# Rutgers-ECE-MML4SS/multimodal-sensor-fusion-with-attention-RajeevAtla

Measured on AMD Instinct MI355X. Metric: HybridFusion fwd+bwd samples/sec at 1/2/4/8 MI355X; CPU-ref parity, higher is better.
Workload: dtype fp32; 1 GPU; c2: HybridFusion M=3 B=256/gpu L=128 D=128 H=128 heads=4 C=5 dropout=0.1 train, fwd+CE(ls=0.05)+bwd+clip(1.0)+AdamW; fused step (flat buffers, one hipGraph); global_batch=256, per_gpu_batch=256, seq_len=128, parallelism=dp1, graph=True, matmul_precision=highest

## Files before the change

multimodal-sensor-fusion-with-attention-rajeevatla_amd/csrc/gemm.hip:

```cpp
#include <algorithm>
#include <cstdlib>
#include <cstring>
#include <map>
#include <vector>

#include "mmf_device.h"

namespace mmf {

namespace {

constexpr int BM = 128, BN = 128, BK = 32, NT = 256;
#ifndef MMF_GEMM_DK
#define MMF_GEMM_DK 16
#endif
#ifndef MMF_GEMM_NS
#define MMF_GEMM_NS 3
#endif
constexpr int LDS_STRIDE = BM + 4;
constexpr int LDS_STRIDE_T = BM + 1;

typedef float f32x4 __attribute__((ext_vector_type(4)));

struct TileCtx {
// ... 1206 lines not shown
  const GemmGroup& g = J.g;
  if (amode != MODE_KR || bmode != MODE_KR || J.nsrc != 1 || !(g.epi & EPI_PARTIAL)) return false;
  if (g.seg_rows > 0 || J.src[0].a.seg_stride || J.src[0].b.seg_stride) return false;
  const int64_t n = (int64_t)(g.nbatch < 1 ? 1 : g.nbatch) * g.nsplit * g.M * (g.N + 1);
  return n <= (1 << 20) && g.kchunk <= 256;
}

struct ReduceArgs {
  ReduceJob j[48];
  int32_t njobs;
};

__global__ __launch_bounds__(256) void partial_reduce_kernel(const ReduceArgs a) {
  ReduceJob J = a.j[blockIdx.y];
  const int64_t MN = (int64_t)J.M * J.N;
  const int batch = blockIdx.z;
  if (batch >= J.nbatch) return;
  J.part += (int64_t)batch * J.nsplit * MN;
  if (J.part_db) J.part_db += (int64_t)batch * J.nsplit * J.M;
  J.out += (int64_t)batch * J.bs_out;
  if (J.db) J.db += (int64_t)batch * J.bs_db;
  __shared__ f32x4 red[4][64];
  const int el = threadIdx.x & 63, sg = threadIdx.x >> 6;
  const bool v4 = (MN % 4) == 0 && ((uintptr_t)J.part & 15) == 0;
  const int64_t n4 = v4 ? MN / 4 : MN;
  const bool out_al = ((uintptr_t)J.out & 15) == 0;
  for (int64_t c0 = (int64_t)blockIdx.x * 64; c0 < n4; c0 += (int64_t)gridDim.x * 64) {
    const int64_t col = c0 + el;
    f32x4 s0 = {0.f, 0.f, 0.f, 0.f}, s1 = s0, s2 = s0, s3 = s0;
    if (col < n4) {
      if (v4) {
        const f32x4* base = reinterpret_cast<const f32x4*>(J.part) + col;
        const int64_t st = MN / 4;
        int k = sg;
#pragma unroll 4
        for (; k + 12 < J.nsplit; k += 16) {
          s0 += base[(int64_t)k * st];
          s1 += base[(int64_t)(k + 4) * st];
          s2 += base[(int64_t)(k + 8) * st];
          s3 += base[(int64_t)(k + 12) * st];
        }
        for (; k < J.nsplit; k += 4) s0 += base[(int64_t)k * st];
      } else {
        for (int k = sg; k < J.nsplit; k += 4) s0[0] += J.part[(int64_t)k * MN + col];
      }
    }
    __syncthreads();
    red[sg][el] = (s0 + s1) + (s2 + s3);
    __syncthreads();
    if (sg == 0 && col < n4) {
      const f32x4 r = (red[0][el] + red[1][el]) + (red[2][el] + red[3][el]);
      if (!v4) J.out[col] = r[0];
      else if (out_al) reinterpret_cast<f32x4*>(J.out)[col] = r;
      else {
        float* o = J.out + col * 4;
        o[0] = r[0]; o[1] = r[1]; o[2] = r[2]; o[3] = r[3];
      }
    }
  }
  if (J.db && (J.part_db || J.nsplit == 0) && blockIdx.x == gridDim.x - 1) {
    __shared__ float redb[4][64];
    for (int i0 = 0; i0 < J.M; i0 += 64) {
      const int i = i0 + el;
      float s0 = 0.f, s1 = 0.f, s2 = 0.f, s3 = 0.f;
      if (i < J.M) {
        int k = sg;
#pragma unroll 4
        for (; k + 12 < J.nsplit; k += 16) {
          s0 += J.part_db[(int64_t)k * J.M + i];
          s1 += J.part_db[(int64_t)(k + 4) * J.M + i];
          s2 += J.part_db[(int64_t)(k + 8) * J.M + i];
          s3 += J.part_db[(int64_t)(k + 12) * J.M + i];
        }
        for (; k < J.nsplit; k += 4) s0 += J.part_db[(int64_t)k * J.M + i];
      }
      __syncthreads();
      redb[sg][el] = (s0 + s1) + (s2 + s3);
      __syncthreads();
      if (sg == 0 && i < J.M) J.db[i] = (redb[0][el] + redb[1][el]) + (redb[2][el] + redb[3][el]);
    }
  }
}

__global__ __launch_bounds__(256) void mask_dropout_rows_kernel(const MaskDropArgs a) {
  const int m = blockIdx.x;
  const bool drop = a.p > 0.f && (a.rng != nullptr || a.rng_live != nullptr);
  RngSnap rs{0, 0};
  {
    const uint64_t* src = a.rng_live ? a.rng_live : (drop ? reinterpret_cast<const uint64_t*>(a.rng) : nullptr);
    if (src) {
      rs.seed = src[0];
      rs.offset = src[1];
    }
  }
  const uint32_t thr = p16(a.p);
  if (m >= a.n) {
    const MaskDropArgs::KeepWordJob& K = a.kw[m - a.n];
    const uint32_t nkt = K.Lk >> 5;
    const uint32_t nwords = (uint32_t)a.B * (uint32_t)a.heads * K.Lq * nkt;
    for (uint32_t i = blockIdx.y * 256u + threadIdx.x; i < nwords; i += gridDim.y * 256u) {
      const uint32_t row = (nkt & (nkt - 1)) == 0 ? i >> (31 - __builtin_clz(nkt)) : i / nkt;
      const uint32_t kt = i - row * nkt;
      const uint64_t blk0 = ((uint64_t)row * K.Lk + 32 * kt) >> 3;
      uint32_t bits = 0;
#pragma unroll
      for (int g = 0; g < 4; ++g) {
        const uint4 rr = philox_block(rs, K.site, blk0 + g);
        const uint32_t wv[4] = {rr.x, rr.y, rr.z, rr.w};
#pragma unroll
        for (int k = 0; k < 4; ++k) {
          bits |= ((wv[k] & 0xFFFFu) >= thr ? 1u : 0u) << (8 * g + 2 * k);
          bits |= ((wv[k] >> 16) >= thr ? 1u : 0u) << (8 * g + 2 * k + 1);
        }
      }
      K.bits[(uint64_t)row * K.kw_ld + kt] = bits;
    }
    return;
  }
  const MaskDropJob& J = a.j[m];
  const int64_t n = J.rows * J.D;
  const float inv_keep = a.p < 1.f ? 1.f / (1.f - a.p) : 0.f;
  const int D = J.D, L = J.L, M = a.M;
  for (int64_t blk = (int64_t)blockIdx.y * blockDim.x + threadIdx.x; blk * 8 < n;
       blk += (int64_t)gridDim.y * blockDim.x) {
    uint4 r = make_uint4(0, 0, 0, 0);
    if (drop) r = philox_block(rs, J.site, (uint64_t)blk);
    const int64_t base = blk * 8;
    if (J.vec && base + 8 <= n) {
      const float sc = a.mask[(base / D / L) * M + m];
      const float4 v0 = *reinterpret_cast<const float4*>(J.x + base);
      const float4 v1 = *reinterpret_cast<const float4*>(J.x + base + 4);
      float o[8] = {v0.x, v0.y, v0.z, v0.w, v1.x, v1.y, v1.z, v1.w};
#pragma unroll
      for (int e = 0; e < 8; ++e) {
        float v = o[e] * sc;
        if (drop) v = keep_from(r, e, thr) ? v * inv_keep : 0.f;
        o[e] = v;
      }
      if (J.outb) {
        bf16x8 pk;
#pragma unroll
        for (int e = 0; e < 8; ++e) pk[e] = (__bf16)o[e];
        *reinterpret_cast<bf16x8*>(reinterpret_cast<__bf16*>(J.out) + base) = pk;
      } else {
        *reinterpret_cast<float4*>(J.out + base) = make_float4(o[0], o[1], o[2], o[3]);
        *reinterpret_cast<float4*>(J.out + base + 4) = make_float4(o[4], o[5], o[6], o[7]);
      }
    } else {
      for (int e = 0; e < 8 && base + e < n; ++e) {
        const int64_t idx = base + e;
        float v = J.x[idx] * a.mask[(idx / D / L) * M + m];
        if (drop) v = keep_from(r, e, thr) ? v * inv_keep : 0.f;
        if (J.outb) reinterpret_cast<__bf16*>(J.out)[idx] = (__bf16)v;
        else J.out[idx] = v;
      }
    }
  }
  if (a.rng_snap && blockIdx.x == 0 && blockIdx.y == 0 && threadIdx.x == 0) *a.rng_snap = rs;
}

bool dma_ok(const Operand& op, int mode, int eext, int bstride, int nbatch) {
  if (!op.vec || op.row_div < 1) return false;
  if (nbatch > 1 && (bstride % 4) != 0) return false;
  if (mode == MODE_KR && (eext % 4) != 0) return false;
  return true;
}

bool job_fast(const GemmJob& J, int amode, int bmode) {
  const GemmGroup& g = J.g;
  const int nb = g.nbatch < 1 ? 1 : g.nbatch;
  if ((g.epi & EPI_PARTIAL) && (g.kchunk % 32) != 0) return false;
  for (int s = 0; s < J.nsrc; ++s) {
    const GemmSrc& src = J.src[s];
    if ((src.K % 4) != 0 || !dma_ok(src.a, amode, g.M, g.bs_a, nb) || !dma_ok(src.b, bmode, g.N, g.bs_b, nb))
      return false;
  }
  return true;
}

}

namespace {

inline bool aligned16(const void* p) { return ((uintptr_t)p & 15) == 0; }

bool job_wsr(const GemmJob& J, int amode, int bmode) {
  const GemmGroup& g = J.g;
  if (amode != MODE_RK || (bmode != MODE_RK && bmode != MODE_KR) || J.nsrc != 1 || g.nbatch > 1) return false;
  if (g.epi & ~(EPI_BIAS | EPI_RELU | EPI_DROP | EPI_COLSUM | EPI_ROWSCALE)) return false;
  static const bool ext_on = getenv("MMF_WSR_EPI") != nullptr;
  if (!ext_on && (bmode != MODE_RK || (g.epi & ~(EPI_BIAS | EPI_RELU)))) return false;
  if ((g.epi & EPI_ROWSCALE) && (g.rs_div <= 0 || g.rs_div % BM != 0 || !g.rowscale)) return false;
  if ((g.epi & EPI_COLSUM) && !g.colsum) return false;
  const GemmSrc& s = J.src[0];
  const bool b_ok = bmode == MODE_RK ? (s.b.ld % 4 == 0 && aligned16(s.b.ptr)) : s.b.ld >= g.N;
  return g.N == BN && g.M % BM == 0 && s.K % WSR_DK == 0 && s.K >= WSR_DK && s.K <= 8 * WSR_NKC &&
         s.a.row_div == 1 && s.b.row_div == 1 && s.a.ld % 4 == 0 && aligned16(s.a.ptr) && b_ok &&
         s.a.seg_stride == 0 && s.b.seg_stride == 0 && g.ldc % 4 == 0 && aligned16(g.C);
}

int cu_count() {
  static int n = 0;
  if (n == 0) {
    int dev = 0;
    if (hipGetDevice(&dev) != hipSuccess ||
        hipDeviceGetAttribute(&n, hipDeviceAttributeMultiprocessorCount, dev) != hipSuccess || n <= 0)
      n = 256;
  }
  return n;
}

hipError_t launch_wsr(const GemmJob* jobs, int njobs, hipStream_t st, uint64_t* rng_advance, int bmode, float drop_p,
                      const RngSnap* rng) {
  for (int done = 0; done < njobs;) {
    GemmArgs args;
    memset(&args, 0, sizeof(args));
    args.amode = MODE_RK;
    args.bmode = bmode;
    args.drop_p = drop_p;
    args.rng = rng;
    args.rng_advance = rng_advance;
    rng_advance = nullptr;
    int ng = 0, items = 0;
    double fl = 0.0, by = 0.0;
    while (done < njobs && ng < GEMM_MAX_GROUPS) {
      GemmGroup g = jobs[done].g;
      g.nbatch = 1;
      g.src_begin = ng;
      g.src_count = 1;
      args.s[ng] = jobs[done].src[0];
      args.tile_off[ng] = items;
      args.g[ng++] = g;
      items += g.M / BM;
      fl += 2.0 * g.M * g.N * jobs[done].src[0].K;
      by += 4.0 * ((double)g.M + g.N) * jobs[done].src[0].K + 4.0 * g.M * g.N;
      ++done;
    }
// ... 468 lines not shown
      GemmGroup g = J.g;
      g.nbatch = 1;
      g.src_begin = ns;
      g.src_count = J.nsrc;
      for (int s = 0; s < J.nsrc; ++s) args.s[ns++] = J.src[s];
      const bool partial = (g.epi & EPI_PARTIAL) != 0;
      args.tile_off[ng] = max_blocks;
      args.g[ng++] = g;
      max_blocks += ((g.M + BM - 1) / BM) * ((g.N + bn - 1) / bn) * (partial ? g.nsplit : 1);
      ++done;
    }
    args.ngroups = ng;
    if (ilv_on && ng > 1) {
      const int T = args.tile_off[1];
      bool even = T > 0 && T % 8 == 0;
      for (int gi = 1; gi < ng && even; ++gi)
        even = (gi + 1 < ng ? args.tile_off[gi + 1] : max_blocks) - args.tile_off[gi] == T;
      args.ilv = even ? 1 : 0;
    }
    double fl = 0.0, by = 0.0;
    for (int gi = 0; gi < ng; ++gi) {
      const GemmGroup& g = args.g[gi];
      const bool partial = (g.epi & EPI_PARTIAL) != 0;
      for (int si = g.src_begin; si < g.src_begin + g.src_count; ++si) {
        fl += 2.0 * g.M * g.N * args.s[si].K;
        by += 2.0 * ((double)g.M + g.N) * args.s[si].K;
      }
      by += partial ? 4.0 * g.nsplit * g.M * g.N
                    : ((g.epi & EPI_BF16) ? 2.0 : 4.0) * g.M * g.N + ((g.epi & EPI_BF16COPY) ? 2.0 * g.M * g.N : 0.0);
    }
    static const char* const kName[4] = {"", "gemm_lds_kernel<0, 0, 32, 3, 1, 1>", "gemm_lds_kernel<1, 1, 32, 3, 1, 2>",
                                         "gemm_lds_kernel<0, 1, 32, 3, 1, 3>"};
    static const char* const kNameW[4] = {"", "", "gemm_lds_kernel<1, 1, 32, 3, 1, 2, 1>",
                                          "gemm_lds_kernel<0, 1, 32, 3, 1, 3, 1>"};
    ProfLaunch prof_(st, wide ? kNameW[form] : kName[form], fl, by);
    if (form == 1) mmf_launch((gemm_lds_kernel<MODE_RK, MODE_RK, 32, 3, 1, 1>), dim3(max_blocks, 1), dim3(NT), 0, st, args);
    else if (form == 2 && wide) mmf_launch((gemm_lds_kernel<MODE_KR, MODE_KR, 32, 3, 1, 2, 1>), dim3(max_blocks, 1), dim3(NT), 0, st, args);
    else if (form == 2) mmf_launch((gemm_lds_kernel<MODE_KR, MODE_KR, 32, 3, 1, 2>), dim3(max_blocks, 1), dim3(NT), 0, st, args);
    else if (wide) mmf_launch((gemm_lds_kernel<MODE_RK, MODE_KR, 32, 3, 1, 3, 1>), dim3(max_blocks, 1), dim3(NT), 0, st, args);
    else mmf_launch((gemm_lds_kernel<MODE_RK, MODE_KR, 32, 3, 1, 3>), dim3(max_blocks, 1), dim3(NT), 0, st, args);
    const hipError_t e = hipGetLastError();
    if (e != hipSuccess) return e;
  }
  return hipSuccess;
}

hipError_t launch_reduce(const ReduceJob* jobs, int njobs, hipStream_t st) {
  int done = 0;
  while (done < njobs) {
    ReduceArgs a;
    memset(&a, 0, sizeof(a));
    int n = 0;
    int64_t maxmn = 0;
    int maxbatch = 1;
    while (done < njobs && n < 48) {
      a.j[n] = jobs[done++];
      if (a.j[n].nbatch < 1) a.j[n].nbatch = 1;
      if (a.j[n].nbatch > maxbatch) maxbatch = a.j[n].nbatch;
      const int64_t mn = (int64_t)a.j[n].M * a.j[n].N;
      if (mn > maxmn) maxmn = mn;
      ++n;
    }
    a.njobs = n;
    int blocks = (int)((maxmn / 4 + 63) / 64);
    if (blocks < 1) blocks = 1;
    if (blocks > 4096) blocks = 4096;
    for (int i = 0; i < n; ++i)
      if (a.j[i].db && (a.j[i].part_db || a.j[i].nsplit == 0)) { ++blocks; break; }
    double by = 0.0;
    for (int i = 0; i < n; ++i) {
      const ReduceJob& r = a.j[i];
      by += 4.0 * r.nbatch * ((double)r.nsplit + 1) * r.M * ((double)r.N + (r.part_db ? 1 : 0));
    }
    ProfLaunch prof_(st, "partial_reduce_kernel", 0.0, by);
    mmf_launch(partial_reduce_kernel, dim3(blocks, n, maxbatch), dim3(256), 0, st, a);
    hipError_t e = hipGetLastError();
    if (e != hipSuccess) return e;
  }
  return hipSuccess;
}

hipError_t launch_mask_dropout(MaskDropArgs a, hipStream_t st) {
  if (a.n < 1 || a.n > 8 || a.nkw < 0 || a.nkw > 16) return hipErrorInvalidValue;
  int64_t maxblk = 1;
  for (int m = 0; m < a.n; ++m) {
    MaskDropJob& J = a.j[m];
    J.vec = (J.D % 8) == 0 && ((uintptr_t)J.x & 15) == 0 && ((uintptr_t)J.out & 15) == 0;
    maxblk = std::max<int64_t>(maxblk, (J.rows * J.D + 7) / 8);
  }
  double by = 0.0;
  for (int m = 0; m < a.n; ++m) by += (a.j[m].outb ? 6.0 : 8.0) * a.j[m].rows * a.j[m].D;
  for (int i = 0; i < a.nkw; ++i) {
    const int64_t nw = (int64_t)a.B * a.heads * a.kw[i].Lq * (a.kw[i].Lk / 32);
    if (a.kw[i].Lk % 32 != 0 || nw >= ((int64_t)1 << 31)) return hipErrorInvalidValue;
    maxblk = std::max<int64_t>(maxblk, nw);
    by += 4.0 * nw;
  }
  const int grid = (int)std::min<int64_t>((maxblk + 255) / 256, 2048);
  ProfLaunch prof_(st, "mask_dropout_rows_kernel", 0.0, by);
  mmf_launch(mask_dropout_rows_kernel, dim3(a.n + a.nkw, grid), dim3(256), 0, st, a);
  return hipGetLastError();
}

}
```

multimodal-sensor-fusion-with-attention-rajeevatla_amd/csrc/mmf_internal.h:

```cpp
#pragma once

#include <hip/hip_runtime.h>
#include <hip/hip_ext.h>
#include <stdint.h>
#include <stddef.h>

namespace mmf {

struct RngSnap { uint64_t seed; uint64_t offset; };

struct ProfArm {
  hipEvent_t a = nullptr, b = nullptr;
  int launches = 0;
};
extern thread_local ProfArm* g_prof_arm;
bool prof_arm_begin(ProfArm& arm, hipStream_t st);
bool prof_capturing(hipStream_t st);

struct SideStream { hipStream_t s; hipEvent_t fork_ev, join_ev; };
SideStream* side_stream(bool create);
void prof_arm_end(ProfArm& arm, hipStream_t st, const char* kernel, double flops, double bytes);
struct ProfLaunch {
  hipStream_t st;
  const char* kernel;
// ... 47 lines not shown
  int32_t seg_stride;
};

struct GemmSrc {
  Operand a, b;
  int32_t K;
  int32_t pad_;
};

enum : int32_t {
  EPI_BIAS = 1, EPI_RELU = 2, EPI_DROP = 4, EPI_ROWADD = 8, EPI_GATE = 16,
  EPI_ROWSCALE = 32, EPI_PARTIAL = 64, EPI_BIAS_RS = 128, EPI_ADDMAT = 256,
  EPI_COLSUM = 512,
  EPI_BF16 = 1024,
  EPI_BF16COPY = 2048,
  EPI_GATE_B16 = 4096
};

struct GemmGroup {
  int32_t M, N;
  int32_t src_begin, src_count;
  float* C; int32_t ldc;
  int32_t epi;
  float alpha;
  const float* bias;
  const float* bias_rs; int32_t bias_rs_ld, bias_rs_off;
  const float* addm; int32_t ld_addm;
  float rowadd_scale;
  const float* rowadd; int32_t ld_rowadd, rowadd_div;
  const float* gate; int32_t ld_gate; float gate_scale;
  const float* rowscale; int32_t rs_div, rs_stride;
  int32_t rs_off;
  uint32_t drop_site;
  int32_t nsplit, kchunk;
  union { float* part_db; float* colsum; };
  int32_t nbatch;
  int32_t bs_a, bs_b, bs_c, bs_bias, bs_brs;
  int32_t seg_rows;
  void* copy;
  int32_t chain;
};

constexpr int GEMM_MAX_GROUPS = 32;
constexpr int GEMM_MAX_SRCS = 32;

struct GemmArgs {
  GemmGroup g[GEMM_MAX_GROUPS];
  GemmSrc s[GEMM_MAX_SRCS];
  int32_t tile_off[GEMM_MAX_GROUPS];
  int32_t ngroups;
  int32_t amode, bmode;
  float drop_p;
  const RngSnap* rng;
  uint64_t* rng_advance;
  int32_t ilv;
};

struct GemmJob {
  GemmGroup g;
  GemmSrc src[GEMM_MAX_SRCS];
  int nsrc;
  const GemmJob* chain;
};

hipError_t launch_gemm(const GemmJob* jobs, int njobs, int amode, int bmode, float drop_p,
                       const RngSnap* rng, hipStream_t st, uint64_t* rng_advance = nullptr);
int device_cu_count();

struct MaskDropJob {
  const float* x; float* out;
  int64_t rows; int32_t D, L;
  uint32_t site; int32_t vec, outb;
};
struct MaskDropArgs {
  MaskDropJob j[8];
  int32_t n, M;
  const float* mask;
  float p;
  const RngSnap* rng;
  const uint64_t* rng_live;
  RngSnap* rng_snap;
  struct KeepWordJob { uint32_t* bits; uint32_t Lq, Lk, kw_ld, site; } kw[16];
  int32_t nkw, B, heads;
};
hipError_t launch_mask_dropout(MaskDropArgs a, hipStream_t st);

struct ReduceJob {
  const float* part; const float* part_db;
  float* out; float* db;
  int32_t nsplit, M, N;
  int32_t nbatch, bs_out, bs_db;
};
hipError_t launch_gemm_b16(const GemmJob* jobs, int njobs, hipStream_t st, int amode = MODE_RK, int bmode = MODE_RK,
                           float drop_p = 0.f, const RngSnap* rng = nullptr, uint64_t* rng_advance = nullptr);
constexpr int CVT_MAX = 72;
struct CvtArgs {
  const float* src[CVT_MAX]; __bf16* dst[CVT_MAX]; float* dst32[CVT_MAX]; int64_t n[CVT_MAX]; int32_t count;
};
hipError_t launch_cvt_bf16(const CvtArgs& a, hipStream_t st);
bool gemm_b16_ok(const GemmJob& J, int amode = MODE_RK, int bmode = MODE_RK);
hipError_t launch_reduce(const ReduceJob* jobs, int njobs, hipStream_t st);

struct AttnPair {
  const float* q; const float* k; const float* v;
  float* o;
  float* lse;
  const float* kmask; int32_t kmask_mode; int32_t kmask_ld;
  int32_t Lq, Lk;
  int32_t ldq, ldk, ldv, ldo;
  uint32_t drop_site;
  const float* dout;
  float* dsum;
  float* dq; float* dk; float* dv;
  float* probs;
  float* pbar;
  float* pbarT;
  const float* dpbar;
  uint32_t* keep_bits;
  int32_t kw_ld;
  float* pstore;
  int32_t qk_bf16;
  int32_t dqk_bf16;
};

constexpr int ATTN_MAX_PAIRS = 12;
inline int64_t attn_pstore_floats(int Lq) { return (int64_t)((Lq + 31) / 32) * 4 * 4 * 64 * 4; }
inline bool attn_pstore_ok(int Lq, int Lk, int kmask_mode, int hd) {
  return Lk % 32 == 0 && Lk <= 128 && Lq <= 128 && kmask_mode != 2 && hd <= 64 && hd % 4 == 0;
}

struct AttnArgs {
  AttnPair p[ATTN_MAX_PAIRS];
  int32_t npairs;
  int32_t B, heads, hd;
  float scale, drop_p;
  int32_t nblk;
  const RngSnap* rng;
};

hipError_t launch_attn_fwd(const AttnPair* pairs, int npairs, int B, int heads, int hd, float scale,
                           float drop_p, const RngSnap* rng, hipStream_t st);
hipError_t launch_attn_probs(const AttnPair* pairs, int npairs, int B, int heads, int hd,
                             float scale, float drop_p, const RngSnap* rng, hipStream_t st);
hipError_t launch_attn_bwd(const AttnPair* pairs, int npairs, int B, int heads, int hd, float scale,
                           float drop_p, const RngSnap* rng, hipStream_t st);
hipError_t launch_attn_bwd_stage(int stage, const AttnPair* pairs, int npairs, int B, int heads, int hd,
                                 float scale, float drop_p, const RngSnap* rng, hipStream_t st);
hipError_t launch_attn_pool_fwd(const AttnPair* pairs, int npairs, int B, int heads, int hd, float scale,
                                float drop_p, const RngSnap* rng, hipStream_t st, bool words_ready = false);
hipError_t launch_attn_pool_bwd(int stage, const AttnPair* pairs, int npairs, int B, int heads, int hd,
                                float scale, float drop_p, const RngSnap* rng, hipStream_t st);
bool attn_long_fused_ok(const AttnPair* pairs, int npairs, int hd, float drop_p);
bool attn_long_fwd_ok(const AttnPair* pairs, int npairs, int hd, float drop_p, const RngSnap* rng);
hipError_t launch_attn_long_fused_fwd(const AttnPair* pairs, int npairs, int B, int heads, int hd, float scale,
                                      float drop_p, const RngSnap* rng, hipStream_t st, bool words_ready = false);
hipError_t launch_attn_keep_words(const AttnPair* pairs, int npairs, int B, int heads, float drop_p,
                                  const RngSnap* rng, hipStream_t st);
hipError_t launch_attn_long_fused_bwd(const AttnPair* pairs, int npairs, int B, int heads, int hd, float scale,
                                      float drop_p, hipStream_t st);

struct SkPair {
  const float* kmask; int32_t kmask_mode; int32_t kmask_ld;
  int32_t Lq;
  uint32_t drop_site;
  float* pbar;
  float* pbarT;
// ... 224 lines not shown
```

multimodal-sensor-fusion-with-attention-rajeevatla_amd/csrc/tail.hip:

```cpp
#include <cstdlib>
#include <cstring>

#include "mmf_device.h"

namespace mmf {

namespace {

constexpr int NT = 256;
constexpr int MAXM = 8;
constexpr int MAXHEADS = 8;

__device__ __forceinline__ float wsum(float v) { return sum64(v); }

template <int S>
__device__ __forceinline__ void gemv_nt_s(const float* xs, int xsamp, int xdiv, int xstride,
                                          const float* __restrict__ W, int N, int K, float* y, int ysamp) {
  const int t = threadIdx.x, half = t & 1;
  const int kh = K >> 1;
  for (int n = t >> 1; n < N; n += NT / 2) {
    const float* x0 = xs + (n / xdiv) * xstride + half * kh;
    const float* w = W + (int64_t)n * K + half * kh;
    float acc[S];
#pragma unroll
// ... 201 lines not shown
  const int H = a.H, nh = a.heads, hd = a.hd, Lk = P.Lk, M = a.M;
  constexpr int DUS = MAXHEADS * TH;
  for (int i = t; i < S * H; i += NT) {
    const int si = i / H, n = i - si * H;
    c_s[si * TH + n] = si < ns ? a.cvec[((int64_t)(b0 + si) * M + P.q) * H + n] : 0.f;
  }
  __syncthreads();
  gemv_nn_s<S>(c_s, TH, P.Wo, H, H, v1, TH, red);
  __syncthreads();
  for (int i = t; i < ns * H; i += NT) {
    const int si = i / H, n = i - si * H;
    P.dOb[(int64_t)(b0 + si) * H + n] = v1[si * TH + n];
  }
  gemv_nn_seg_s<S>(v1, TH, P.Wv, nh, hd, H, du_s, DUS);
  for (int sh = wave; sh < S * nh; sh += NT / 64) {
    const int si = sh / nh, hh = sh - si * nh;
    float s = 0.f;
    for (int d = lane; d < hd; d += 64) s += v1[si * TH + hh * hd + d] * P.bv[hh * hd + d];
    s = wsum(s);
    if (lane == 0) dr_s[si * MAXHEADS + hh] = s;
  }
  __syncthreads();
  for (int i = t; i < ns * nh * H; i += NT) {
    const int si = i / (nh * H), r = i - si * nh * H;
    P.dU[(int64_t)(b0 + si) * nh * H + r] = du_s[si * DUS + r];
  }
  const int half = lane >> 5, l32 = lane & 31;
  for (int si = 0; si < ns; ++si) {
    const int b = b0 + si;
    const float* pk = P.Pk + (int64_t)b * Lk * H;
    const float* du = du_s + si * DUS;
#pragma unroll 2
    for (int j0 = 2 * wave; j0 < Lk; j0 += 2 * (NT / 64)) {
      const int j = j0 + half;
      float acc[MAXHEADS];
#pragma unroll
      for (int hh = 0; hh < MAXHEADS; ++hh) acc[hh] = 0.f;
      if (j < Lk) {
        for (int c4 = l32; c4 < H / 4; c4 += 32) {
          const float4 v = *reinterpret_cast<const float4*>(pk + (int64_t)j * H + 4 * c4);
#pragma unroll
          for (int hh = 0; hh < MAXHEADS; ++hh) {
            if (hh < nh) {
              const float4 u = *reinterpret_cast<const float4*>(&du[hh * H + 4 * c4]);
              acc[hh] += v.x * u.x + v.y * u.y + v.z * u.z + v.w * u.w;
            }
          }
        }
      }
#pragma unroll
      for (int hh = 0; hh < MAXHEADS; ++hh) {
        if (hh < nh) {
          const float sv = sum32(acc[hh]);
          if (l32 == 0 && j < Lk) P.dpbar[((int64_t)b * nh + hh) * Lk + j] = sv + dr_s[si * MAXHEADS + hh];
        }
      }
    }
  }
}

constexpr int KG_ROWS = 32;

__device__ __forceinline__ float4 ld4(const float* p) { return *reinterpret_cast<const float4*>(p); }

__device__ __forceinline__ f32x16 mfma4(const float4& a, const float4& b, f32x16 acc) {
  acc = mfma32(a.x, b.x, acc);
  acc = mfma32(a.y, b.y, acc);
  acc = mfma32(a.z, b.z, acc);
  return mfma32(a.w, b.w, acc);
}

__device__ __forceinline__ f32x16 zero16() {
  f32x16 z;
#pragma unroll
  for (int r = 0; r < 16; ++r) z[r] = 0.f;
  return z;
}

__global__ __launch_bounds__(NT, 3) void tail_u_kernel(const TailArgs a) {
  constexpr int PS = 128 + 4;
  constexpr int RPT = 16;
  __shared__ __attribute__((aligned(16))) float pb_s[KG_ROWS * PS];
  __shared__ __attribute__((aligned(16))) float4 red4[8 * NT];
  const int b = blockIdx.x, kg = blockIdx.y;
  const int t = threadIdx.x, lane = t & 63, w = t >> 6;
  const int H = a.H, nh = a.heads, R = a.kg_cnt[kg] * nh, H4 = H >> 2, RG = NT / H4;
  const int c4 = t % H4, rg = t / H4;
  const TailPair& P0 = a.p[a.kg_pair[kg][0]];
  const int Lk = P0.Lk;
  const float* pk = P0.Pk + (int64_t)b * Lk * H + 4 * c4;
  float4 v[RPT];
  auto load_rows = [&](int j0) {
#pragma unroll
    for (int i = 0; i < RPT; ++i) {
      const int j = j0 + rg + RG * i;
      v[i] = ld4(pk + (int64_t)min(j, Lk - 1) * H);
    }
  };
  load_rows(0);
  const int per = nh * Lk;
  if (per % 64 == 0) {
    constexpr int U = 4;
    for (int i0 = 0; i0 < R * Lk; i0 += U * NT) {
      float vv[U];
#pragma unroll
      for (int u = 0; u < U; ++u) {
        const int i = min(i0 + u * NT + t, R * Lk - 1);
        const int slot = __builtin_amdgcn_readfirstlane(i / per);
        vv[u] = a.p[a.kg_pair[kg][slot]].pbar[(int64_t)b * per + (i - slot * per)];
      }
#pragma unroll
      for (int u = 0; u < U; ++u) {
        const int i = i0 + u * NT + t;
        if (i < R * Lk) {
          const int row = i / Lk, j = i - row * Lk;
          pb_s[row * PS + j] = vv[u];
        }
      }
    }
  } else {
    for (int i = t; i < R * Lk; i += NT) {
      const int row = i / Lk, j = i - row * Lk;
      pb_s[row * PS + j] = a.p[a.kg_pair[kg][row / nh]].pbar[((int64_t)b * nh + row % nh) * Lk + j];
    }
  }
  __syncthreads();
  for (int row = w; row < R; row += NT / 64) {
    float s = 0.f;
    for (int j = lane; j < Lk; j += 64) s += pb_s[row * PS + j];
    s = wsum(s);
    if (lane == 0) a.p[a.kg_pair[kg][row / nh]].r[(int64_t)b * nh + row % nh] = s;
  }
  for (int r0 = 0; r0 < R; r0 += 8) {
    float4 acc[8];
#pragma unroll
    for (int rr = 0; rr < 8; ++rr) acc[rr] = make_float4(0.f, 0.f, 0.f, 0.f);
    for (int j0 = 0; j0 < Lk; j0 += RG * RPT) {
      if (j0 > 0) load_rows(j0);
#pragma unroll
      for (int i = 0; i < RPT; ++i) {
        const int j = j0 + rg + RG * i;
        if (j < Lk) {
#pragma unroll
          for (int rr = 0; rr < 8; ++rr) {
            if (r0 + rr < R) {
              const float wgt = pb_s[(r0 + rr) * PS + j];
              acc[rr].x += wgt * v[i].x; acc[rr].y += wgt * v[i].y;
              acc[rr].z += wgt * v[i].z; acc[rr].w += wgt * v[i].w;
            }
          }
        }
      }
    }
    if (R > 8 && Lk > RG * RPT) load_rows(0);
#pragma unroll
    for (int rr = 0; rr < 8; ++rr) red4[rr * NT + t] = acc[rr];
    __syncthreads();
    for (int task = t; task < 8 * H4; task += NT) {
      const int rr = task / H4, cc = task - rr * H4;
      if (r0 + rr < R) {
        float4 s = red4[rr * NT + cc];
        for (int g = 1; g < RG; ++g) {
          const float4 u = red4[rr * NT + g * H4 + cc];
          s.x += u.x; s.y += u.y; s.z += u.z; s.w += u.w;
        }
        const int row = r0 + rr;
        *reinterpret_cast<float4*>(a.p[a.kg_pair[kg][row / nh]].U + ((int64_t)b * nh + row % nh) * H + 4 * cc) = s;
      }
    }
    __syncthreads();
  }
}

constexpr int NTW = 512;
constexpr int WH = 128;

__device__ __forceinline__ f32x16 mfma8(const float4 (&a)[8], const float4 (&b)[8], f32x16 acc) {
#pragma unroll
  for (int q = 0; q < 8; ++q) acc = mfma4(a[q], b[q], acc);
  return acc;
}

__device__ __forceinline__ void split_reduce(float (*part)[16][64], f32x16& acc, int kq, int ts, int lane) {
  if (kq == 1) {
#pragma unroll
    for (int r = 0; r < 16; ++r) part[ts][r][lane] = acc[r];
  }
  __syncthreads();
  if (kq == 0) {
#pragma unroll
    for (int r = 0; r < 16; ++r) acc[r] += part[ts][r][lane];
  }
}

__global__ __launch_bounds__(NTW) void tail_ob_mfma_kernel(const TailArgs a) {
  constexpr int OS = WH + 4;
  __shared__ __attribute__((aligned(16))) float ob_s[32 * OS];
  __shared__ float part[4][16][64];
  const TailPair& P = a.p[blockIdx.y];
  const int s0 = blockIdx.x * 32;
  const int t = threadIdx.x, lane = t & 63, w = t >> 6, hf = lane >> 5, c = lane & 31;
  const int ts = w & 3, kq = w >> 2, k0 = kq * 64 + 4 * hf;
  const int nh = a.heads, hd = a.hd, B = a.B;
  const int sa = min(s0 + c, B - 1);
  const int n = ts * 32 + c, hh = (ts * 32) / hd;
  float4 au[8], bv[8], bo[8];
  const float* urow = P.U + ((int64_t)sa * nh + hh) * WH + k0;
  const float* vrow = P.Wv + (int64_t)n * WH + k0;
  const float* orow = P.Wo + (int64_t)n * WH + k0;
#pragma unroll
  for (int q = 0; q < 8; ++q) {
    au[q] = ld4(urow + 8 * q);
    bv[q] = ld4(vrow + 8 * q);
    bo[q] = ld4(orow + 8 * q);
  }
  float rs[16];
#pragma unroll
  for (int r = 0; r < 16; ++r) {
    const int s = s0 + acc_row(r, hf);
    rs[r] = P.r[(int64_t)min(s, B - 1) * nh + hh];
  }
  const float bvn = P.bv[n], bon = P.bo[n];
  __builtin_amdgcn_sched_barrier(0);
  f32x16 acc = mfma8(au, bv, zero16());
  split_reduce(part, acc, kq, ts, lane);
  if (kq == 0) {
#pragma unroll
    for (int r = 0; r < 16; ++r) {
      const int i = acc_row(r, hf), s = s0 + i;
      const float o = acc[r] + rs[r] * bvn;
      ob_s[i * OS + n] = o;
      if (s < B) P.Ob[(int64_t)s * WH + n] = o;
    }
  }
  __syncthreads();
  float4 ao[8];
#pragma unroll
  for (int q = 0; q < 8; ++q) ao[q] = ld4(ob_s + c * OS + k0 + 8 * q);
  acc = mfma8(ao, bo, zero16());
  split_reduce(part, acc, kq, ts, lane);
  if (kq == 0) {
#pragma unroll
    for (int r = 0; r < 16; ++r) {
      const int s = s0 + acc_row(r, hf);
      if (s < B) P.Ab[(int64_t)s * WH + n] = acc[r] + bon;
    }
  }
}

__global__ __launch_bounds__(NTW) void tail_dob_mfma_kernel(const TailArgs a) {
  constexpr int OS = WH + 4;
  __shared__ __attribute__((aligned(16))) float dob_s[32 * OS];
  __shared__ float part[4][16][64];
  const TailPair& P = a.p[blockIdx.y];
  const int s0 = blockIdx.x * 32;
  const int t = threadIdx.x, lane = t & 63, w = t >> 6, hf = lane >> 5, c = lane & 31;
  const int ts = w & 3, kq = w >> 2, k0 = kq * 64 + 4 * hf;
  const int nh = a.heads, hd = a.hd, B = a.B, M = a.M;
  const int sa = min(s0 + c, B - 1);
  const int n = ts * 32 + c;
  float4 ac[8], bw[8];
  const float* crow = a.cvec + ((int64_t)sa * M + P.q) * WH + k0;
  const float* wcol = P.Wo + (int64_t)k0 * WH + n;
#pragma unroll
  for (int q = 0; q < 8; ++q) {
    ac[q] = ld4(crow + 8 * q);
    bw[q] = make_float4(wcol[(8 * q) * WH], wcol[(8 * q + 1) * WH], wcol[(8 * q + 2) * WH], wcol[(8 * q + 3) * WH]);
  }
  const int ntile = nh * (WH / 32);
  float4 bu[2][8];
#pragma unroll
  for (int u = 0; u < 2; ++u) {
    const int tt = w + 8 * u;
    const int hh = tt >> 2, kc = (tt & 3) * 32 + c;
    const float* vcol = P.Wv + (int64_t)(hh * hd + 4 * hf) * WH + kc;
#pragma unroll
    for (int q = 0; q < 8; ++q) {
      bu[u][q] = make_float4(0.f, 0.f, 0.f, 0.f);
      if (tt < ntile && 8 * q < hd)
        bu[u][q] = make_float4(vcol[(8 * q) * WH], vcol[(8 * q + 1) * WH], vcol[(8 * q + 2) * WH],
                               vcol[(8 * q + 3) * WH]);
    }
  }
  f32x16 acc = mfma8(ac, bw, zero16());
  split_reduce(part, acc, kq, ts, lane);
  if (kq == 0) {
#pragma unroll
    for (int r = 0; r < 16; ++r) {
      const int i = acc_row(r, hf), s = s0 + i;
      dob_s[i * OS + n] = acc[r];
      if (s < B) P.dOb[(int64_t)s * WH + n] = acc[r];
    }
  }
  __syncthreads();
#pragma unroll
  for (int u = 0; u < 2; ++u) {
    const int tt = w + 8 * u;
    if (tt >= ntile) break;
    const int hh = tt >> 2, kc = (tt & 3) * 32 + c;
    f32x16 acc2 = zero16();
#pragma unroll
    for (int q = 0; q < 8; ++q)
      if (8 * q < hd) acc2 = mfma4(ld4(dob_s + c * OS + hh * hd + 4 * hf + 8 * q), bu[u][q], acc2);
#pragma unroll
    for (int r = 0; r < 16; ++r) {
      const int s = s0 + acc_row(r, hf);
      if (s < B) P.dU[((int64_t)s * nh + hh) * WH + kc] = acc2[r];
    }
  }
}

__global__ __launch_bounds__(NT) void tail_dpbar_mfma_kernel(const TailArgs a) {
  __shared__ __attribute__((aligned(16))) float du_s[KG_ROWS * (TAIL_MAX_H + 4)];
  __shared__ float dr_s[KG_ROWS];
  __shared__ float* rowp[KG_ROWS];
  const int b = blockIdx.x, kg = blockIdx.y;
  const int t = threadIdx.x, lane = t & 63, w = t >> 6, hf = lane >> 5, c = lane & 31;
  const int H = a.H, nh = a.heads, hd = a.hd, R = a.kg_cnt[kg] * nh, DS = H + 4;
  const TailPair& P0 = a.p[a.kg_pair[kg][0]];
  const int Lk = P0.Lk;
  const float* pk = P0.Pk + (int64_t)b * Lk * H;
  float4 av[16];
  auto load_a = [&](int mt, int k0) {
    const float* arow = pk + (int64_t)min(mt * 32 + c, Lk - 1) * H + k0 + 4 * hf;
#pragma unroll
    for (int q = 0; q < 16; ++q)
      if (k0 + 8 * q < H) av[q] = ld4(arow + 8 * q);
  };
  if (w * 32 < Lk) load_a(w, 0);
  const int H4 = H / 4, per = nh * H4;
  if (per % 64 == 0) {
    constexpr int U = 4;
    for (int i0 = 0; i0 < KG_ROWS * H4; i0 += U * NT) {
      float4 vv[U];
#pragma unroll
      for (int u = 0; u < U; ++u) {
        const int i = min(i0 + u * NT + t, R * H4 - 1);
        const int slot = __builtin_amdgcn_readfirstlane(i / per);
        const int e = i - slot * per;
        vv[u] = ld4(a.p[a.kg_pair[kg][slot]].dU + (int64_t)b * nh * H + 4 * e);
      }
#pragma unroll
      for (int u = 0; u < U; ++u) {
        const int i = i0 + u * NT + t;
        if (i < KG_ROWS * H4) {
          const int row = i / H4, c4 = (i - row * H4) * 4;
          const float4 q = row < R ? vv[u] : make_float4(0.f, 0.f, 0.f, 0.f);
          reinterpret_cast<f32x4v*>(du_s)[(row * DS + c4) >> 2] = f32x4v{q.x, q.y, q.z, q.w};
        }
      }
    }
  } else {
    for (int i = t; i < KG_ROWS * H4; i += NT) {
      const int row = i / H4, c4 = (i - row * H4) * 4;
      float4 v = make_float4(0.f, 0.f, 0.f, 0.f);
      if (row < R) v = ld4(a.p[a.kg_pair[kg][row / nh]].dU + ((int64_t)b * nh + row % nh) * H + c4);
      reinterpret_cast<f32x4v*>(du_s)[(row * DS + c4) >> 2] = f32x4v{v.x, v.y, v.z, v.w};
    }
  }
  if (t < R) rowp[t] = a.p[a.kg_pair[kg][t / nh]].dpbar + ((int64_t)b * nh + t % nh) * Lk;
  for (int row = w; row < R; row += NT / 64) {
    const TailPair& P = a.p[a.kg_pair[kg][row / nh]];
    const int hh = row % nh;
    float s = 0.f;
    for (int d = lane; d < hd; d += 64) s += P.dOb[(int64_t)b * H + hh * hd + d] * P.bv[hh * hd + d];
    s = wsum(s);
    if (lane == 0) dr_s[row] = s;
  }
  __syncthreads();
  const float* brow = du_s + c * DS + 4 * hf;
  for (int mt = w; mt * 32 < Lk; mt += NT / 64) {
    f32x16 acc = zero16();
    for (int k0 = 0; k0 < H; k0 += 128) {
      if (mt != w || k0 > 0) load_a(mt, k0);
#pragma unroll
      for (int q = 0; q < 16; ++q)
        if (k0 + 8 * q < H) acc = mfma4(av[q], ld4(brow + k0 + 8 * q), acc);
    }
    if (c < R) {
      float* outp = rowp[c];
      const float dr = dr_s[c];
#pragma unroll
      for (int r = 0; r < 16; ++r) {
        const int kk = mt * 32 + acc_row(r, hf);
        if (kk < Lk) outp[kk] = acc[r] + dr;
      }
    }
  }
}

constexpr int PH = 128;

__device__ __forceinline__ void gemv128_pre(const float* x, const float4 (&wr)[16], float* y) {
  const int t = threadIdx.x, half = t & 1;
  const float* x0 = x + half * 64;
  float acc = 0.f;
#pragma unroll
  for (int q = 0; q < 16; ++q) {
    const float4 xv = *reinterpret_cast<const float4*>(x0 + 4 * q);
    acc += wr[q].x * xv.x + wr[q].y * xv.y + wr[q].z * xv.z + wr[q].w * xv.w;
  }
  const float v = acc + dpp<DPP_XOR1>(acc);
  if (half == 0) y[t >> 1] = v;
}

template <int NW>
__device__ __forceinline__ void gemv_nn128_pre(const float* x, const float (&wc)[NW], int n0, int cnt, float* y,
                                               float* red) {
  const int t = threadIdx.x;
  float acc = 0.f;
#pragma unroll
  for (int i = 0; i < NW; ++i)
    if (i < cnt) acc += x[n0 + i] * wc[i];
  red[t] = acc;
  __syncthreads();
  if (t < 128) y[t] = red[t] + red[t + 128];
}

template <bool PRE>
__global__ __launch_bounds__(NT) void tail_head_fwd_kernel(const TailArgs a) {
  __shared__ __attribute__((aligned(16))) float pooled_s[MAXM * TAIL_MAX_H];
  __shared__ __attribute__((aligned(16))) float v1[TAIL_MAX_H], v2[TAIL_MAX_H];
  __shared__ __attribute__((aligned(16))) float4 red4[NT];
  __shared__ float score_s[MAXM], w_s[MAXM];
  const int b = blockIdx.x;
  const int t = threadIdx.x, lane = t & 63, wave = __builtin_amdgcn_readfirstlane(t >> 6);
  const int M = a.M, H = a.H;
  const int H4 = H >> 2;
  float4 w1r[16];
  float gw[2] = {0.f, 0.f}, w2r[2][2] = {{0.f, 0.f}, {0.f, 0.f}}, b1n = 0.f;
  if constexpr (PRE) {
    const float* wr = a.W1 + (int64_t)(t >> 1) * PH + (t & 1) * 64;
#pragma unroll
    for (int q = 0; q < 16; ++q) w1r[q] = *reinterpret_cast<const float4*>(wr + 4 * q);
    if (wave < M) {
      gw[0] = a.gate_w[wave][lane];
      gw[1] = a.gate_w[wave][lane + 64];
    }
#pragma unroll
    for (int u = 0; u < 2; ++u)
      if (wave + 4 * u < a.C) {
        w2r[u][0] = a.W2[(int64_t)(wave + 4 * u) * PH + lane];
        w2r[u][1] = a.W2[(int64_t)(wave + 4 * u) * PH + lane + 64];
      }
    if (t < PH) b1n = a.b1[t];
  }
  if constexpr (PRE) {
    constexpr int PM = 4, PG = 12;
    const int n = t;
    if (n < H) {
// ... 386 lines not shown
```

Baseline: 273,900 samples/s.

## Unroll mask-dropout loads and reorder tail kernel loads for latency overlap

The mask/dropout kernel now handles two 256-element chunks per thread iteration. It issues all global loads before any compute, uses a 32-bit divide for the mask index, and sizes the row and keep-word grids independently so unused blocks exit early. In the tail pbar and dpbar kernels, per-row output pointers are precomputed into shared memory. The Pk and dOb/bv register loads are moved to issue alongside the first batch of shared-memory staging loads, fenced by sched barriers, to overlap global memory latency. The changes raise register pressure and touch several kernels at once.

New measurement: 275,000 samples/s (median of 6 runs). No clear change (+0.4%).

```diff
diff --git a/multimodal-sensor-fusion-with-attention-rajeevatla_amd/csrc/gemm.hip b/multimodal-sensor-fusion-with-attention-rajeevatla_amd/csrc/gemm.hip
--- a/multimodal-sensor-fusion-with-attention-rajeevatla_amd/csrc/gemm.hip
+++ b/multimodal-sensor-fusion-with-attention-rajeevatla_amd/csrc/gemm.hip
@@ -1312,8 +1312,50 @@
   }
 }
 
+constexpr int MASK_U = 2;
+constexpr int MASK_KWT = 2;
+
+__device__ __forceinline__ void mask_drop_block(const MaskDropArgs& a, const MaskDropJob& J, int m, int64_t blk,
+                                                int64_t n, bool drop, const RngSnap& rs, uint32_t thr,
+                                                float inv_keep) {
+  const int D = J.D, L = J.L, M = a.M;
+  uint4 r = make_uint4(0, 0, 0, 0);
+  if (drop) r = philox_block(rs, J.site, (uint64_t)blk);
+  const int64_t base = blk * 8;
+  if (J.vec && base + 8 <= n) {
+    const float sc = a.mask[(base / D / L) * M + m];
+    const float4 v0 = *reinterpret_cast<const float4*>(J.x + base);
+    const float4 v1 = *reinterpret_cast<const float4*>(J.x + base + 4);
+    float o[8] = {v0.x, v0.y, v0.z, v0.w, v1.x, v1.y, v1.z, v1.w};
+#pragma unroll
+    for (int e = 0; e < 8; ++e) {
+      float v = o[e] * sc;
+      if (drop) v = keep_from(r, e, thr) ? v * inv_keep : 0.f;
+      o[e] = v;
+    }
+    if (J.outb) {
+      bf16x8 pk;
+#pragma unroll
+      for (int e = 0; e < 8; ++e) pk[e] = (__bf16)o[e];
+      *reinterpret_cast<bf16x8*>(reinterpret_cast<__bf16*>(J.out) + base) = pk;
+    } else {
+      *reinterpret_cast<float4*>(J.out + base) = make_float4(o[0], o[1], o[2], o[3]);
+      *reinterpret_cast<float4*>(J.out + base + 4) = make_float4(o[4], o[5], o[6], o[7]);
+    }
+  } else {
+    for (int e = 0; e < 8 && base + e < n; ++e) {
+      const int64_t idx = base + e;
+      float v = J.x[idx] * a.mask[(idx / D / L) * M + m];
+      if (drop) v = keep_from(r, e, thr) ? v * inv_keep : 0.f;
+      if (J.outb) reinterpret_cast<__bf16*>(J.out)[idx] = (__bf16)v;
+      else J.out[idx] = v;
+    }
+  }
+}
+
 __global__ __launch_bounds__(256) void mask_dropout_rows_kernel(const MaskDropArgs a) {
   const int m = blockIdx.x;
+  if ((int)blockIdx.y >= (m >= a.n ? a.kw_chunks : a.row_chunks)) return;
   const bool drop = a.p > 0.f && (a.rng != nullptr || a.rng_live != nullptr);
   RngSnap rs{0, 0};
   {
@@ -1328,7 +1370,7 @@
     const MaskDropArgs::KeepWordJob& K = a.kw[m - a.n];
     const uint32_t nkt = K.Lk >> 5;
     const uint32_t nwords = (uint32_t)a.B * (uint32_t)a.heads * K.Lq * nkt;
-    for (uint32_t i = blockIdx.y * 256u + threadIdx.x; i < nwords; i += gridDim.y * 256u) {
+    for (uint32_t i = blockIdx.y * 256u + threadIdx.x; i < nwords; i += (uint32_t)a.kw_chunks * 256u) {
       const uint32_t row = (nkt & (nkt - 1)) == 0 ? i >> (31 - __builtin_clz(nkt)) : i / nkt;
       const uint32_t kt = i - row * nkt;
       const uint64_t blk0 = ((uint64_t)row * K.Lk + 32 * kt) >> 3;
@@ -1350,39 +1392,50 @@
   const MaskDropJob& J = a.j[m];
   const int64_t n = J.rows * J.D;
   const float inv_keep = a.p < 1.f ? 1.f / (1.f - a.p) : 0.f;
-  const int D = J.D, L = J.L, M = a.M;
-  for (int64_t blk = (int64_t)blockIdx.y * blockDim.x + threadIdx.x; blk * 8 < n;
-       blk += (int64_t)gridDim.y * blockDim.x) {
-    uint4 r = make_uint4(0, 0, 0, 0);
-    if (drop) r = philox_block(rs, J.site, (uint64_t)blk);
-    const int64_t base = blk * 8;
-    if (J.vec && base + 8 <= n) {
-      const float sc = a.mask[(base / D / L) * M + m];
-      const float4 v0 = *reinterpret_cast<const float4*>(J.x + base);
-      const float4 v1 = *reinterpret_cast<const float4*>(J.x + base + 4);
-      float o[8] = {v0.x, v0.y, v0.z, v0.w, v1.x, v1.y, v1.z, v1.w};
-#pragma unroll
-      for (int e = 0; e < 8; ++e) {
-        float v = o[e] * sc;
-        if (drop) v = keep_from(r, e, thr) ? v * inv_keep : 0.f;
-        o[e] = v;
-      }
-      if (J.outb) {
-        bf16x8 pk;
-#pragma unroll
-        for (int e = 0; e < 8; ++e) pk[e] = (__bf16)o[e];
-        *reinterpret_cast<bf16x8*>(reinterpret_cast<__bf16*>(J.out) + base) = pk;
-      } else {
-        *reinterpret_cast<float4*>(J.out + base) = make_float4(o[0], o[1], o[2], o[3]);
-        *reinterpret_cast<float4*>(J.out + base + 4) = make_float4(o[4], o[5], o[6], o[7]);
+  const int64_t DL = (int64_t)J.D * J.L;
+  const bool fast = J.vec && n <= 0xFFFFFFFFll && DL <= 0xFFFFFFFFll && DL > 0;
+  constexpr int64_t SPAN = (int64_t)MASK_U * 256;
+  for (int64_t blk0 = (int64_t)blockIdx.y * SPAN; blk0 * 8 < n; blk0 += (int64_t)a.row_chunks * SPAN) {
+    if (fast && (blk0 + SPAN) * 8 <= n) {
+      float4 v[MASK_U][2];
+      float sc[MASK_U];
+#pragma unroll
+      for (int u = 0; u < MASK_U; ++u) {
+        const int64_t base = (blk0 + u * 256 + threadIdx.x) * 8;
+        v[u][0] = *reinterpret_cast<const float4*>(J.x + base);
+        v[u][1] = *reinterpret_cast<const float4*>(J.x + base + 4);
+      }
+#pragma unroll
+      for (int u = 0; u < MASK_U; ++u) {
+        const uint32_t base = (uint32_t)((blk0 + u * 256 + threadIdx.x) * 8);
+        sc[u] = a.mask[(int64_t)(base / (uint32_t)DL) * a.M + m];
+      }
+#pragma unroll
+      for (int u = 0; u < MASK_U; ++u) {
+        const int64_t blk = blk0 + u * 256 + threadIdx.x, base = blk * 8;
+        uint4 r = make_uint4(0, 0, 0, 0);
+        if (drop) r = philox_block(rs, J.site, (uint64_t)blk);
+        float o[8] = {v[u][0].x, v[u][0].y, v[u][0].z, v[u][0].w, v[u][1].x, v[u][1].y, v[u][1].z, v[u][1].w};
+#pragma unroll
+        for (int e = 0; e < 8; ++e) {
+          float x = o[e] * sc[u];
+          if (drop) x = keep_from(r, e, thr) ? x * inv_keep : 0.f;
+          o[e] = x;
+        }
+        if (J.outb) {
+          bf16x8 pk;
+#pragma unroll
+          for (int e = 0; e < 8; ++e) pk[e] = (__bf16)o[e];
+          *reinterpret_cast<bf16x8*>(reinterpret_cast<__bf16*>(J.out) + base) = pk;
+        } else {
+          *reinterpret_cast<float4*>(J.out + base) = make_float4(o[0], o[1], o[2], o[3]);
+          *reinterpret_cast<float4*>(J.out + base + 4) = make_float4(o[4], o[5], o[6], o[7]);
+        }
       }
     } else {
-      for (int e = 0; e < 8 && base + e < n; ++e) {
-        const int64_t idx = base + e;
-        float v = J.x[idx] * a.mask[(idx / D / L) * M + m];
-        if (drop) v = keep_from(r, e, thr) ? v * inv_keep : 0.f;
-        if (J.outb) reinterpret_cast<__bf16*>(J.out)[idx] = (__bf16)v;
-        else J.out[idx] = v;
+      for (int u = 0; u < MASK_U; ++u) {
+        const int64_t blk = blk0 + u * 256 + threadIdx.x;
+        if (blk * 8 < n) mask_drop_block(a, J, m, blk, n, drop, rs, thr, inv_keep);
       }
     }
   }
@@ -2017,7 +2070,7 @@
 
 hipError_t launch_mask_dropout(MaskDropArgs a, hipStream_t st) {
   if (a.n < 1 || a.n > 8 || a.nkw < 0 || a.nkw > 16) return hipErrorInvalidValue;
-  int64_t maxblk = 1;
+  int64_t maxblk = 1, maxkw = 0;
   for (int m = 0; m < a.n; ++m) {
     MaskDropJob& J = a.j[m];
     J.vec = (J.D % 8) == 0 && ((uintptr_t)J.x & 15) == 0 && ((uintptr_t)J.out & 15) == 0;
@@ -2028,10 +2081,12 @@
   for (int i = 0; i < a.nkw; ++i) {
     const int64_t nw = (int64_t)a.B * a.heads * a.kw[i].Lq * (a.kw[i].Lk / 32);
     if (a.kw[i].Lk % 32 != 0 || nw >= ((int64_t)1 << 31)) return hipErrorInvalidValue;
-    maxblk = std::max<int64_t>(maxblk, nw);
+    maxkw = std::max<int64_t>(maxkw, nw);
     by += 4.0 * nw;
   }
-  const int grid = (int)std::min<int64_t>((maxblk + 255) / 256, 2048);
+  a.row_chunks = (int)std::min<int64_t>((maxblk + MASK_U * 256 - 1) / (MASK_U * 256), 2048);
+  a.kw_chunks = (int)std::min<int64_t>((maxkw + MASK_KWT * 256 - 1) / (MASK_KWT * 256), 2048);
+  const int grid = std::max(a.row_chunks, a.kw_chunks);
   ProfLaunch prof_(st, "mask_dropout_rows_kernel", 0.0, by);
   mmf_launch(mask_dropout_rows_kernel, dim3(a.n + a.nkw, grid), dim3(256), 0, st, a);
   return hipGetLastError();
diff --git a/multimodal-sensor-fusion-with-attention-rajeevatla_amd/csrc/mmf_internal.h b/multimodal-sensor-fusion-with-attention-rajeevatla_amd/csrc/mmf_internal.h
--- a/multimodal-sensor-fusion-with-attention-rajeevatla_amd/csrc/mmf_internal.h
+++ b/multimodal-sensor-fusion-with-attention-rajeevatla_amd/csrc/mmf_internal.h
@@ -153,6 +153,7 @@
   RngSnap* rng_snap;
   struct KeepWordJob { uint32_t* bits; uint32_t Lq, Lk, kw_ld, site; } kw[16];
   int32_t nkw, B, heads;
+  int32_t row_chunks, kw_chunks;
 };
 hipError_t launch_mask_dropout(MaskDropArgs a, hipStream_t st);
 
diff --git a/multimodal-sensor-fusion-with-attention-rajeevatla_amd/csrc/tail.hip b/multimodal-sensor-fusion-with-attention-rajeevatla_amd/csrc/tail.hip
--- a/multimodal-sensor-fusion-with-attention-rajeevatla_amd/csrc/tail.hip
+++ b/multimodal-sensor-fusion-with-attention-rajeevatla_amd/csrc/tail.hip
@@ -307,6 +307,7 @@
   constexpr int RPT = 16;
   __shared__ __attribute__((aligned(16))) float pb_s[KG_ROWS * PS];
   __shared__ __attribute__((aligned(16))) float4 red4[8 * NT];
+  __shared__ float* up_s[KG_ROWS];
   const int b = blockIdx.x, kg = blockIdx.y;
   const int t = threadIdx.x, lane = t & 63, w = t >> 6;
   const int H = a.H, nh = a.heads, R = a.kg_cnt[kg] * nh, H4 = H >> 2, RG = NT / H4;
@@ -314,6 +315,10 @@
   const TailPair& P0 = a.p[a.kg_pair[kg][0]];
   const int Lk = P0.Lk;
   const float* pk = P0.Pk + (int64_t)b * Lk * H + 4 * c4;
+  for (int g = 0; g < a.kg_cnt[kg]; ++g) {
+    float* up = a.p[a.kg_pair[kg][g]].U;
+    if (t < R && t / nh == g) up_s[t] = up + ((int64_t)b * nh + t % nh) * H;
+  }
   float4 v[RPT];
   auto load_rows = [&](int j0) {
 #pragma unroll
@@ -322,7 +327,6 @@
       v[i] = ld4(pk + (int64_t)min(j, Lk - 1) * H);
     }
   };
-  load_rows(0);
   const int per = nh * Lk;
   if (per % 64 == 0) {
     constexpr int U = 4;
@@ -334,6 +338,11 @@
         const int slot = __builtin_amdgcn_readfirstlane(i / per);
         vv[u] = a.p[a.kg_pair[kg][slot]].pbar[(int64_t)b * per + (i - slot * per)];
       }
+      if (i0 == 0) {
+        __builtin_amdgcn_sched_barrier(0);
+        load_rows(0);
+        __builtin_amdgcn_sched_barrier(0);
+      }
 #pragma unroll
       for (int u = 0; u < U; ++u) {
         const int i = i0 + u * NT + t;
@@ -344,6 +353,7 @@
       }
     }
   } else {
+    load_rows(0);
     for (int i = t; i < R * Lk; i += NT) {
       const int row = i / Lk, j = i - row * Lk;
       pb_s[row * PS + j] = a.p[a.kg_pair[kg][row / nh]].pbar[((int64_t)b * nh + row % nh) * Lk + j];
@@ -354,7 +364,8 @@
     float s = 0.f;
     for (int j = lane; j < Lk; j += 64) s += pb_s[row * PS + j];
     s = wsum(s);
-    if (lane == 0) a.p[a.kg_pair[kg][row / nh]].r[(int64_t)b * nh + row % nh] = s;
+    const int slot = __builtin_amdgcn_readfirstlane(row / nh);
+    if (lane == 0) a.p[a.kg_pair[kg][slot]].r[(int64_t)b * nh + row % nh] = s;
   }
   for (int r0 = 0; r0 < R; r0 += 8) {
     float4 acc[8];
@@ -389,8 +400,7 @@
           const float4 u = red4[rr * NT + g * H4 + cc];
           s.x += u.x; s.y += u.y; s.z += u.z; s.w += u.w;
         }
-        const int row = r0 + rr;
-        *reinterpret_cast<float4*>(a.p[a.kg_pair[kg][row / nh]].U + ((int64_t)b * nh + row % nh) * H + 4 * cc) = s;
+        *reinterpret_cast<float4*>(up_s[r0 + rr] + 4 * cc) = s;
       }
     }
     __syncthreads();
@@ -545,6 +555,10 @@
   const TailPair& P0 = a.p[a.kg_pair[kg][0]];
   const int Lk = P0.Lk;
   const float* pk = P0.Pk + (int64_t)b * Lk * H;
+  for (int g = 0; g < a.kg_cnt[kg]; ++g) {
+    float* dp = a.p[a.kg_pair[kg][g]].dpbar;
+    if (t < R && t / nh == g) rowp[t] = dp + ((int64_t)b * nh + t % nh) * Lk;
+  }
   float4 av[16];
   auto load_a = [&](int mt, int k0) {
     const float* arow = pk + (int64_t)min(mt * 32 + c, Lk - 1) * H + k0 + 4 * hf;
@@ -552,7 +566,19 @@
     for (int q = 0; q < 16; ++q)
       if (k0 + 8 * q < H) av[q] = ld4(arow + 8 * q);
   };
-  if (w * 32 < Lk) load_a(w, 0);
+  constexpr int DRR = KG_ROWS / (NT / 64);
+  const bool dr_pre = hd <= 64;
+  float dob_r[DRR], bv_r[DRR];
+  auto load_dr = [&]() {
+#pragma unroll
+    for (int i = 0; i < DRR; ++i) {
+      const int row = min(w + (NT / 64) * i, R - 1);
+      const TailPair& P = a.p[a.kg_pair[kg][__builtin_amdgcn_readfirstlane(row / nh)]];
+      const int e = (row % nh) * hd + min(lane, hd - 1);
+      dob_r[i] = P.dOb[(int64_t)b * H + e];
+      bv_r[i] = P.bv[e];
+    }
+  };
   const int H4 = H / 4, per = nh * H4;
   if (per % 64 == 0) {
     constexpr int U = 4;
@@ -564,6 +590,12 @@
         const int slot = __builtin_amdgcn_readfirstlane(i / per);
         const int e = i - slot * per;
         vv[u] = ld4(a.p[a.kg_pair[kg][slot]].dU + (int64_t)b * nh * H + 4 * e);
+      }
+      if (i0 == 0) {
+        load_dr();
+        __builtin_amdgcn_sched_barrier(0);
+        if (w * 32 < Lk) load_a(w, 0);
+        __builtin_amdgcn_sched_barrier(0);
       }
 #pragma unroll
       for (int u = 0; u < U; ++u) {
@@ -576,6 +608,8 @@
       }
     }
   } else {
+    load_dr();
+    if (w * 32 < Lk) load_a(w, 0);
     for (int i = t; i < KG_ROWS * H4; i += NT) {
       const int row = i / H4, c4 = (i - row * H4) * 4;
       float4 v = make_float4(0.f, 0.f, 0.f, 0.f);
@@ -583,14 +617,24 @@
       reinterpret_cast<f32x4v*>(du_s)[(row * DS + c4) >> 2] = f32x4v{v.x, v.y, v.z, v.w};
     }
   }
-  if (t < R) rowp[t] = a.p[a.kg_pair[kg][t / nh]].dpbar + ((int64_t)b * nh + t % nh) * Lk;
-  for (int row = w; row < R; row += NT / 64) {
-    const TailPair& P = a.p[a.kg_pair[kg][row / nh]];
-    const int hh = row % nh;
-    float s = 0.f;
-    for (int d = lane; d < hd; d += 64) s += P.dOb[(int64_t)b * H + hh * hd + d] * P.bv[hh * hd + d];
-    s = wsum(s);
-    if (lane == 0) dr_s[row] = s;
+  if (dr_pre) {
+#pragma unroll
+    for (int i = 0; i < DRR; ++i) {
+      const int row = w + (NT / 64) * i;
+      if (row < R) {
+        const float s = wsum(lane < hd ? 0.f + dob_r[i] * bv_r[i] : 0.f);
+        if (lane == 0) dr_s[row] = s;
+      }
+    }
+  } else {
+    for (int row = w; row < R; row += NT / 64) {
+      const TailPair& P = a.p[a.kg_pair[kg][row / nh]];
+      const int hh = row % nh;
+      float s = 0.f;
+      for (int d = lane; d < hd; d += 64) s += P.dOb[(int64_t)b * H + hh * hd + d] * P.bv[hh * hd + d];
+      s = wsum(s);
+      if (lane == 0) dr_s[row] = s;
+    }
   }
   __syncthreads();
   const float* brow = du_s + c * DS + 4 * hf;
```
